# samuel-watson/glmmrMCML

Measured on AMD Instinct MI355X. Metric: MCML iters/sec x m chains (simlik evals/sec), higher is better.
Workload: dtype f64

## Files before the change

glmmrmcml_amd/csrc/dgemm_band.h:

```cpp
#pragma once
#include "dgemm_dlds.h"
#include "band_plan.h"

namespace mcml {

struct BandP {
    GemmP g;
    const BandItem* items;
    const int* wg_ptr;
    int nwg;
    double* part;
    int mode;
    unsigned long long* clocks;
};

static __global__ __launch_bounds__(256) void k_band_ranges(const double* A, int lda, int M, int K, int* krange)
{
    __shared__ int smin[256], smax[256];
    const int band = blockIdx.x, r0 = band * BD_BM;
    const int rows = (M - r0 < BD_BM) ? (M - r0) : BD_BM;
    int kmin = 1 << 30, kmax = -1;
    for (int k = threadIdx.x; k < K; k += 256) {
        const double* col = A + r0 + (size_t)k * lda;
        bool nz = false;
        for (int r = 0; r < rows; ++r) nz |= (col[r] != 0.0);
        if (nz) { kmin = min(kmin, k); kmax = max(kmax, k); }
    }
    smin[threadIdx.x] = kmin; smax[threadIdx.x] = kmax;
    __syncthreads();
    for (int o = 128; o > 0; o >>= 1) {
        if ((int)threadIdx.x < o) {
            smin[threadIdx.x] = min(smin[threadIdx.x], smin[threadIdx.x + o]);
            smax[threadIdx.x] = max(smax[threadIdx.x], smax[threadIdx.x + o]);
        }
        __syncthreads();
    }
    if (threadIdx.x == 0) {
        if (smax[0] < 0) { krange[2 * band] = 0; krange[2 * band + 1] = 0; }
        else { krange[2 * band] = smin[0] / BD_BK; krange[2 * band + 1] = smax[0] / BD_BK + 1; }
    }
}

#if defined(__HIP_DEVICE_COMPILE__)
#define BD_RD(dst, addr, off) asm volatile("ds_read_b64 %0, %1 offset:%2" : "=v"(dst) : "v"(addr), "i"(off))
#else
#define BD_RD(dst, addr, off) (dst = 0.0)
#endif
template <int KS, int NS>
__device__ __forceinline__ void bd_read(double (&a)[5], double (&b)[NS], unsigned aaddr, unsigned baddr)
{
    static_assert(NS == 1 || NS == 2, "one or two strips per wave");
    BD_RD(a[0], aaddr, KS * 4 * BD_BM * 8);
    BD_RD(a[1], aaddr, KS * 4 * BD_BM * 8 + 128);
    BD_RD(a[2], aaddr, KS * 4 * BD_BM * 8 + 256);
    BD_RD(a[3], aaddr, KS * 4 * BD_BM * 8 + 384);
    BD_RD(a[4], aaddr, KS * 4 * BD_BM * 8 + 512);
    BD_RD(b[0], baddr, KS * 2 * BD_BN * 16);
    if constexpr (NS == 2) BD_RD(b[1], baddr, KS * 2 * BD_BN * 16 + 256);
}
template <int LEAVE, int NS>
__device__ __forceinline__ void bd_wait(double (&a)[5], double (&b)[NS])
{
    static_assert(LEAVE == 0 || LEAVE == 5 + NS, "one substep's reads");
#if defined(__HIP_DEVICE_COMPILE__)
    if constexpr (NS == 1)
        asm volatile("s_waitcnt lgkmcnt(%[n])" : "+v"(a[0]), "+v"(a[1]), "+v"(a[2]), "+v"(a[3]), "+v"(a[4]), "+v"(b[0]) : [n] "n"(LEAVE));
    else
        asm volatile("s_waitcnt lgkmcnt(%[n])" : "+v"(a[0]), "+v"(a[1]), "+v"(a[2]), "+v"(a[3]), "+v"(a[4]), "+v"(b[0]), "+v"(b[1]) : [n] "n"(LEAVE));
#endif
}
template <int NS>
__device__ __forceinline__ void bd_mfma(d4 (&acc)[NS][5][1], const double (&a)[5], const double (&b)[NS])
{
#pragma unroll
    for (int j = 0; j < NS; ++j)
#pragma unroll
        for (int i = 0; i < 5; ++i) acc[j][i][0] = __builtin_amdgcn_mfma_f64_16x16x4f64(b[j], a[i], acc[j][i][0], 0, 0, 0);
}

__device__ __forceinline__ BandItem band_item(const BandItem* ip)
{
    BandItem item{0, 0, 0, -1};
#if defined(__HIP_DEVICE_COMPILE__)
    typedef int i4s __attribute__((ext_vector_type(4)));
    i4s raw;
    asm volatile("s_load_dwordx4 %0, %1, 0x0\n\ts_waitcnt lgkmcnt(0)" : "=&s"(raw) : "s"(ip) : "memory");
    item.band = raw.x; item.kt0 = raw.y; item.kt1 = raw.z; item.slot = raw.w;
#else
    item = *ip;
#endif
    return item;
}

template <int STRIDE, int NA, int NB>
struct BandFill {
    static constexpr int PER_TILE = NA + NB, A_CHUNKS = BD_A_BYTES / 1024;
    static_assert(STRIDE * NA >= A_CHUNKS && STRIDE * NB * 1024 == BD_B_BYTES, "the role's waves cover a stage");
    const GemmP& p;
    const BandItem* items;
    const int f, lane;
    const unsigned lds0;
    const size_t stepA;
    unsigned voa[NA], vob[NB];
    const char* sA = nullptr; const char* sB = nullptr;
    BandItem item{0, 0, 0, -1};

    __device__ __forceinline__ int a_rel(int s) const
    {
        return (STRIDE * NA > A_CHUNKS && f + STRIDE * s >= A_CHUNKS) ? STRIDE : STRIDE * s;
    }
    __device__ __forceinline__ BandFill(const BandP& bp, int f_, int lane_, int n0, unsigned lds0_)
        : p(bp.g), items(bp.items), f(f_), lane(lane_), lds0(lds0_), stepA((size_t)BD_BK * bp.g.lda * 8)
    {
#pragma unroll
        for (int s = 0; s < NB; ++s) {
            const int c = f + STRIDE * s;
            const int kp = c >> 1, n = ((c & 1) << 6) + lane;
            int gn = n0 + n;
            if (gn >= p.N) gn = 0;
            vob[s] = (unsigned)((2 * kp + (size_t)gn * p.ldb) * 8);
        }
    }
    __device__ __forceinline__ void load_item(int it)
    {
        item = band_item(items + it);
        const int m0 = item.band * BD_BM;
#pragma unroll
        for (int s = 0; s < NA; ++s) {
            const int o = (f + a_rel(s)) * 1024 + lane * 16;
            const int k = o / (BD_BM * 8), m = (o - k * BD_BM * 8) >> 3;
            int gm = m0 + m;
            if (gm >= p.M) gm = 0;
            voa[s] = (unsigned)((gm + (size_t)k * p.lda) * 8);
        }
        sA = reinterpret_cast<const char*>(p.A) + (size_t)item.kt0 * stepA;
        sB = reinterpret_cast<const char*>(p.B) + (size_t)item.kt0 * (BD_BK * 8);
    }
    __device__ __forceinline__ void issue(int stage)
    {
        const unsigned lbase = lds0 + stage * BD_STAGE_BYTES + f * 1024;
#pragma unroll
        for (int s = 0; s < NA; ++s) lds_dma16(lbase + a_rel(s) * 1024, voa[s], sA);
#pragma unroll
        for (int s = 0; s < NB; ++s) lds_dma16(lbase + BD_A_BYTES + STRIDE * s * 1024, vob[s], sB);
        sA += stepA;
        sB += BD_BK * 8;
    }
    __device__ __forceinline__ void wait_leave(int tiles) const
    {
        if (tiles >= 2) asm volatile("s_waitcnt vmcnt(%0)" :: "n"(2 * PER_TILE) : "memory");
        else if (tiles == 1) asm volatile("s_waitcnt vmcnt(%0)" :: "n"(PER_TILE) : "memory");
        else asm volatile("s_waitcnt vmcnt(0)" ::: "memory");
    }
};
struct BandNoFill {
    const BandItem* items;
    BandItem item{0, 0, 0, -1};
    __device__ __forceinline__ BandNoFill(const BandP& bp, int, int, int, unsigned) : items(bp.items) {}
    __device__ __forceinline__ void load_item(int it) { item = band_item(items + it); }
    __device__ __forceinline__ void issue(int) {}
    __device__ __forceinline__ void wait_leave(int) const {}
};
constexpr int BF_NA = 5, BF_NB = 8;

__device__ __forceinline__ void band_store_partial(double* tile, int strip, int lane, const d4 (&acc)[5][1])
{
    double* P = tile + (size_t)strip * (20 * 64) + lane;
#pragma unroll
    for (int i = 0; i < 5; ++i)
#pragma unroll
        for (int r = 0; r < 4; ++r) P[(i * 4 + r) * 64] = acc[i][0][r];
}

struct BandWg {
    int wave, lane, bj, it0, it1;
    __device__ __forceinline__ explicit BandWg(const BandP& bp)
    {
        const int tid = threadIdx.x;
        lane = tid & 63;
        wave = __builtin_amdgcn_readfirstlane(tid >> 6);
        const int nid = xcd_block_map(blockIdx.x, bp.nwg * bp.g.gn);
        const int pw = nid / bp.g.gn;
        bj = nid - pw * bp.g.gn;
        it0 = bp.wg_ptr[pw]; it1 = bp.wg_ptr[pw + 1];
    }
};

template <int NS, class Fill, bool DBG, class Epi>
__device__ __forceinline__ void band_walk(const BandP& bp, const Epi& epi, const BandWg& wg, int piece0, int strip0)
{
    constexpr int NJ = NS > 0 ? NS : 1;
    const GemmP& p = bp.g;
    extern __shared__ __attribute__((aligned(16))) double smem[];
    const unsigned lds0 = (unsigned)(size_t)(lds_ptr_t) reinterpret_cast<char*>(smem);
    const int lane = wg.lane, l15 = lane & 15, lk = lane >> 4;
    const int bj = wg.bj, n0 = bj * BD_BN, it0 = wg.it0, it1 = wg.it1;

    auto stamp = [&](int i) {
        if constexpr (DBG)
            if ((bp.mode & 16) && bp.clocks && threadIdx.x == 0)
                bp.clocks[8 + 8 * (size_t)blockIdx.x + i] = __builtin_amdgcn_s_memrealtime();
    };
    stamp(0);
    bool first_item = true;
    Fill fill(bp, piece0, lane, n0, lds0);
    bool pre = false;
    int issued = 0;
    if (it0 < it1) fill.load_item(it0);
    for (int it = it0; it < it1;) {
        const int band = fill.item.band, slot = fill.item.slot;
        const int nk = fill.item.kt1 - fill.item.kt0;

        d4 acc[NJ][5][1];
#pragma unroll
        for (int j = 0; j < NJ; ++j)
#pragma unroll
            for (int i = 0; i < 5; ++i) acc[j][i][0] = d4{0.0, 0.0, 0.0, 0.0};

        if (nk > 0) {
            const unsigned aoff = lds0 + lk * (BD_BM * 8) + l15 * 8;
            const unsigned boff = lds0 + BD_A_BYTES + (((lk >> 1) * BD_BN + strip0 * 16 + l15) << 4) + ((lk & 1) << 3);
            if (!pre) { issued = 0; for (; issued < BD_STAGES - 1 && issued < nk; ++issued) fill.issue(issued); }
            fill.wait_leave(issued - 1);
            __builtin_amdgcn_s_barrier();
            if (first_item) stamp(1);
            int st = 0;
            double ra[2][5], rb[2][NJ];
            if constexpr (NS > 0) bd_read<0>(ra[0], rb[0], aoff, boff);
            for (int kt = 0; kt < nk; ++kt) {
                if (issued < nk) {
                    int sn = st + BD_STAGES - 1; if (sn >= BD_STAGES) sn -= BD_STAGES;
                    fill.issue(sn);
                    ++issued;
                }
                const unsigned aaddr = aoff + st * BD_STAGE_BYTES, baddr = boff + st * BD_STAGE_BYTES;
                int stn = st + 1; if (stn >= BD_STAGES) stn = 0;
                if constexpr (NS > 0) {
#define BD_STEP(KS, CUR, NXT)                                   \
                    bd_read<KS + 1>(ra[NXT], rb[NXT], aaddr, baddr); \
                    bd_wait<5 + NS>(ra[CUR], rb[CUR]);               \
                    bd_mfma(acc, ra[CUR], rb[CUR]);                  \
                    __builtin_amdgcn_sched_barrier(0);
                    BD_STEP(0, 0, 1) BD_STEP(1, 1, 0) BD_STEP(2, 0, 1) BD_STEP(3, 1, 0)
                    BD_STEP(4, 0, 1) BD_STEP(5, 1, 0) BD_STEP(6, 0, 1)
#undef BD_STEP
                }
                fill.wait_leave(issued - kt - 2);
                if constexpr (NS > 0) bd_wait<0>(ra[1], rb[1]);
                __builtin_amdgcn_s_barrier();
                if constexpr (NS > 0) {
                    if (kt + 1 < nk) bd_read<0>(ra[0], rb[0], aoff + stn * BD_STAGE_BYTES, boff + stn * BD_STAGE_BYTES);
                    bd_mfma(acc, ra[1], rb[1]);
                    __builtin_amdgcn_sched_barrier(0);
                }
                st = stn;
            }
        }
        if (first_item) stamp(2);
        ++it;
        pre = false;
        if (it < it1) {
            fill.load_item(it);
            const int nkn = fill.item.kt1 - fill.item.kt0;
            if (nk > 0 && nkn > 0) {
                issued = 0;
                for (; issued < BD_STAGES - 1 && issued < nkn; ++issued) fill.issue(issued);
                pre = true;
            }
        }
        if constexpr (NS > 0) {
            if (slot < 0) {
                int elane = lane;
                if constexpr (NS > 1) asm volatile("" : "+v"(elane));
                epi(acc[0], band * BD_BM, n0 + strip0 * 16, elane, p.M, p.N, band);
                if constexpr (NS > 1) {
                    __builtin_amdgcn_sched_barrier(0);
                    epi(acc[1], band * BD_BM, n0 + strip0 * 16 + 16, elane, p.M, p.N, band);
                }
            } else {
                double* tile = bp.part + ((size_t)slot * p.gn + bj) * BD_TILE_ELEMS;
#pragma unroll
                for (int j = 0; j < NS; ++j) band_store_partial(tile, strip0 + j, lane, acc[j]);
            }
        }
        if (first_item) { stamp(3); first_item = false; }
        if (!pre) __builtin_amdgcn_s_barrier();
    }
    if constexpr (DBG)
        if ((bp.mode & 16) && bp.clocks) { asm volatile("s_waitcnt vmcnt(0)" ::: "memory"); stamp(4); }
}

template <class Epi, bool DBG>
__global__ __launch_bounds__(512) void dgemm_band_kernel(BandP bp, Epi epi)
{
    const BandWg wg(bp);
    unsigned long long t0c = 0, t0r = 0;
    if constexpr (DBG)
        if (bp.clocks && blockIdx.x == 0 && threadIdx.x == 0) { t0c = __builtin_amdgcn_s_memtime(); t0r = __builtin_amdgcn_s_memrealtime(); }
    band_walk<1, BandFill<8, BD_NA, BD_NB>, DBG>(bp, epi, wg, wg.wave, wg.wave);
    if constexpr (DBG)
        if (bp.clocks && blockIdx.x == 0 && threadIdx.x == 0) {
            atomicAdd(bp.clocks, __builtin_amdgcn_s_memtime() - t0c);
            atomicAdd(bp.clocks + 1, __builtin_amdgcn_s_memrealtime() - t0r);
        }
}

template <class Epi> struct BandFeed { static constexpr bool ok = false; };
template <> struct BandFeed<EpiAxpby> { static constexpr bool ok = true; };

static inline bool band_feed_enabled()
{
    const char* e = getenv("GLMMR_MCML_BAND_FEED");
    return !(e && !strcmp(e, "0"));
}

template <class Epi>
__global__ __launch_bounds__(512) void dgemm_band_feed_kernel(BandP bp, Epi epi)
{
    const BandWg wg(bp);
    if (wg.wave >= 4) band_walk<0, BandFill<4, BF_NA, BF_NB>, false>(bp, epi, wg, wg.wave - 4, 0);
    else band_walk<2, BandNoFill, false>(bp, epi, wg, 0, 2 * wg.wave);
}

template <class Epi>
__global__ __launch_bounds__(128) void k_band_reduce(const BandRed* red, const double* part, int gn, int M, int N, Epi epi)
{
    const BandRed rd = red[blockIdx.x];
    const int bj = blockIdx.y;
    const int lane = threadIdx.x & 63, wave = blockIdx.z * 2 + (threadIdx.x >> 6);
    d4 acc[5][1];
#pragma unroll
    for (int i = 0; i < 5; ++i) acc[i][0] = d4{0.0, 0.0, 0.0, 0.0};
    const size_t pstride = (size_t)gn * BD_TILE_ELEMS;
    const double* P0 = part + ((size_t)rd.s0 * gn + bj) * BD_TILE_ELEMS + (size_t)wave * (20 * 64) + lane;
    for (int s = rd.s0; s < rd.s1; s += 4) {
        double v[4][20];
#pragma unroll
        for (int u = 0; u < 4; ++u) {
            const double* P = P0 + (size_t)(s - rd.s0 + (s + u < rd.s1 ? u : 0)) * pstride;
#pragma unroll
            for (int t = 0; t < 20; ++t) v[u][t] = P[t * 64];
        }
#pragma unroll
        for (int u = 0; u < 4; ++u)
            if (s + u < rd.s1) {
#pragma unroll
                for (int i = 0; i < 5; ++i)
#pragma unroll
                    for (int r = 0; r < 4; ++r) acc[i][0][r] += v[u][i * 4 + r];
            }
    }
    epi(acc, rd.band * BD_BM, bj * BD_BN + wave * 16, lane, M, N, rd.band);
}

enum { BAND_FORM_AUTO = -1, BAND_FORM_8WAVE = 0, BAND_FORM_FEED = 1 };
template <class Epi, bool DBG = false>
static inline int launch_gemm_band(hipStream_t s, BandPlan& plan, int N, const double* A, int lda,
                                   const double* B, int ldb, const Epi& epi,
                                   unsigned long long* clocks = nullptr, int mode = 0, int form = BAND_FORM_AUTO,
                                   int* whole_band = nullptr)
{
    const int gn = (N + BD_BN - 1) / BD_BN;
    BandPlanDev* d = nullptr;
    MCML_TRY(plan.device_plan(gn, s, &d));
    BandP bp;
    bp.clocks = clocks;
    bp.mode = mode;
    bp.g = GemmP{plan.M, N, plan.K, A, lda, B, ldb, 0, gn, 0};
    bp.items = d->items.as<BandItem>();
    bp.wg_ptr = d->wg_ptr.as<int>();
    bp.nwg = d->nwg;
    bp.part = d->part.d();
    if (whole_band) *whole_band = d->paired;
    bool feed = false;
    if constexpr (BandFeed<Epi>::ok && !DBG) {
        feed = form == BAND_FORM_AUTO ? band_feed_enabled() : form == BAND_FORM_FEED;
        if (feed) {
            MCML_TRY(ensure_dynamic_lds(reinterpret_cast<const void*>(&dgemm_band_feed_kernel<Epi>), (int)BD_LDS_BYTES));
            hipLaunchKernelGGL((dgemm_band_feed_kernel<Epi>), dim3(d->nwg * gn), dim3(512), BD_LDS_BYTES, s, bp, epi);
        }
    }
    MCML_REQUIRE(feed || form != BAND_FORM_FEED, "launch_gemm_band: no feeder form of this instantiation");
    if (!feed) {
        MCML_TRY(ensure_dynamic_lds(reinterpret_cast<const void*>(&dgemm_band_kernel<Epi, DBG>), (int)BD_LDS_BYTES));
        hipLaunchKernelGGL((dgemm_band_kernel<Epi, DBG>), dim3(d->nwg * gn), dim3(512), BD_LDS_BYTES, s, bp, epi);
    }
    if (d->nred > 0)
        hipLaunchKernelGGL((k_band_reduce<Epi>), dim3(d->nred, gn, 4), dim3(128), 0, s, d->red.as<BandRed>(),
                           d->part.d(), gn, plan.M, N, epi);
    MCML_HIP(hipGetLastError());
    return MCML_OK;
}


}
```

glmmrmcml_amd/csrc/hmc.hip:

```cpp
#include <algorithm>
#include <atomic>
#include <chrono>
#include "entry.h"
#include "dgemm_mfma.h"
#include "dgemm_dlds.h"
#include "dgemm_band.h"
#include "dgemm_skinny.h"
#include "glm.h"
#include "reduce.h"
#include "rng.h"
#include "hmc_chain.h"
#include "hmc_cm.h"
#include "hmc_traj.h"

namespace mcml {

template <int FL>
struct EpiForwardT {
    double* MU; double* S; int ld; const double* xb; const double* y; int flink; int store_mu; double var_par;
    __device__ __forceinline__ double score(double yv, double mu) const {
        if constexpr (FL == 12) return glm_score_beta(yv, mu, var_par);
        else return glm_score(yv, mu, FL ? FL : flink);
    }
    __device__ __forceinline__ void elem(int m, int n, double accv) const {
        const double mu = xb[m] + accv;
        if (store_mu) MU[m + (size_t)n * ld] = mu;
        S[m + (size_t)n * ld] = score(y[m], mu);
    }
    template <int TM, int TN>
    __device__ __forceinline__ void operator()(d4 (&acc)[TM][TN], int mB, int nB, int lane, int M, int N,
                                               int) const {
        double xbv[TM], yv[TM];
#pragma unroll
        for (int i = 0; i < TM; ++i) {
            const int m = mB + 16 * i + (lane & 15);
            const int mm = m < M ? m : 0;
            xbv[i] = xb[mm]; yv[i] = y[mm];
        }
        double sc[TM][TN][4];
#pragma unroll
        for (int i = 0; i < TM; ++i)
#pragma unroll
            for (int j = 0; j < TN; ++j)
#pragma unroll
                for (int r = 0; r < 4; ++r) {
                    const double mu = xbv[i] + acc[i][j][r];
                    acc[i][j][r] = mu;
                    sc[i][j][r] = score(yv[i], mu);
                }
#pragma unroll
        for (int j = 0; j < TN; ++j)
#pragma unroll
            for (int r = 0; r < 4; ++r) {
                const int n = nB + 16 * j + (lane >> 4) + 4 * r;
                if (n >= N) continue;
#pragma unroll
                for (int i = 0; i < TM; ++i) {
                    const int m = mB + 16 * i + (lane & 15);
                    if (m < M) {
                        if (store_mu) MU[m + (size_t)n * ld] = acc[i][j][r];
                        S[m + (size_t)n * ld] = sc[i][j][r];
                    }
                }
            }
    }
};

struct EpiBackward {
    const double* Xs; double* G; double* R; double* UP; int ld;
    const double* e; const int* steps; int s; double post; int mode;
    __device__ __forceinline__ void elem(int m, int n, double accv) const {
        int st = 0; double en = 0.0;
        if (mode == 1) { st = steps[n]; en = e[n]; if (s >= st) return; }
        const size_t off = m + (size_t)n * ld;
        const double x = Xs[off];
        double g = -1.0 * x;
        g = g + post * accv;
        if (mode != 1 || s + 1 >= st) G[off] = g;
        if (mode == 1) {
            double rr = R[off];
            rr = rr + (en / 2) * g;
            if (s + 1 < st) {
                rr = rr + (en / 2) * g;
                UP[off] = x + en * rr;
            }
            R[off] = rr;
        }
    }
    template <int TM, int TN>
    __device__ __forceinline__ void operator()(d4 (&acc)[TM][TN], int mB, int nB, int lane, int M, int N,
                                               int) const {
#pragma unroll
        for (int j = 0; j < TN; ++j) {
            int stv[4]; double env[4]; bool inN[4]; size_t cb[4];
#pragma unroll
            for (int r = 0; r < 4; ++r) {
                const int n = nB + 16 * j + (lane >> 4) + 4 * r;
                inN[r] = n < N;
                const int nn = inN[r] ? n : 0;
                stv[r] = mode == 1 ? steps[nn] : 0;
                env[r] = mode == 1 ? e[nn] : 0.0;
                cb[r] = (size_t)nn * ld;
            }
            double xv[TM][4], rv[TM][4];
#pragma unroll
            for (int i = 0; i < TM; ++i) {
                const int m = mB + 16 * i + (lane & 15);
                const int mm = m < M ? m : 0;
#pragma unroll
                for (int r = 0; r < 4; ++r) {
                    xv[i][r] = Xs[mm + cb[r]];
                    rv[i][r] = mode == 1 ? R[mm + cb[r]] : 0.0;
                }
            }
#pragma unroll
            for (int r = 0; r < 4; ++r) {
                const double en = env[r];
                const bool more = s + 1 < stv[r];
#pragma unroll
                for (int i = 0; i < TM; ++i) {
                    const double x = xv[i][r];
                    double g = -1.0 * x;
                    g = g + post * acc[i][j][r];
                    acc[i][j][r] = g;
                    double rr = rv[i][r];
                    rr = rr + (en / 2) * g;
                    const double rr2 = rr + (en / 2) * g;
                    rr = more ? rr2 : rr;
                    rv[i][r] = rr;
                    xv[i][r] = x + en * rr;
                }
            }
#pragma unroll
            for (int r = 0; r < 4; ++r) {
                const bool act = inN[r] && (mode != 1 || s < stv[r]);
                if (!act) continue;
                const bool more = s + 1 < stv[r];
#pragma unroll
                for (int i = 0; i < TM; ++i) {
                    const int m = mB + 16 * i + (lane & 15);
                    if (m >= M) continue;
                    const size_t off = m + cb[r];
                    if (mode != 1 || !more) G[off] = acc[i][j][r];
                    if (mode == 1) {
                        if (more) UP[off] = xv[i][r];
                        R[off] = rv[i][r];
                    }
                }
            }
        }
    }
};

template <> struct BandFeed<EpiBackward> { static constexpr bool ok = true; };
template <> struct BandFeed<EpiForwardT<1>> { static constexpr bool ok = true; };
template <> struct BandFeed<EpiForwardT<3>> { static constexpr bool ok = true; };
template <> struct BandFeed<EpiForwardT<7>> { static constexpr bool ok = true; };


__global__ __launch_bounds__(256) void k_blockdiag_LV(int Q, int ncols, const int* start, const double* L, int ldl,
                                                      const double* V, int ldv, double* U, int ldu)
{
    const int q = blockIdx.x * 256 + threadIdx.x;
    if (q >= Q) return;
    const int s0 = start[q];
    for (int c = blockIdx.y; c < ncols; c += gridDim.y) {
        const double* v = V + (size_t)c * ldv;
        double acc = 0.0;
        for (int t = s0; t <= q; ++t) acc += L[q + (size_t)t * ldl] * v[t];
        U[q + (size_t)c * ldu] = acc;
    }
}

__global__ __launch_bounds__(256) void k_hmc_init(double* V, int ld, int Q, ChainArrays ca, uint64_t seed,
                                                  uint32_t chain_offset, uint32_t iter_idx, const double* inj_init)
{
    const int c = blockIdx.x;
    const uint32_t gid = chain_offset + (uint32_t)c;
    for (int q = threadIdx.x; q < Q; q += 256)
        V[q + (size_t)c * ld] = inj_init ? inj_init[q + (size_t)c * Q]
                                         : rng_normal(seed, (uint32_t)q, gid, 0u, 16u * iter_idx + 0u);
    if (threadIdx.x == 0) chain_reset(ca, c, seed, gid, iter_idx);
}

template <int FL>
__device__ __forceinline__ double chain_log_prob(const double* MU, int ldm, int n, const double* X, int ldx,
                                                 int Q, const double* y, double var_par, int flink_rt, int c,
                                                 double* sh)
{
    const int flink = FL ? FL : flink_rt;
    double ll = 0, lp = 0;
    for (int i0 = threadIdx.x; i0 < n; i0 += 1024) {
        double m4[4], y4[4];
#pragma unroll
        for (int u = 0; u < 4; ++u) {
            const int i = i0 + 256 * u;
            m4[u] = i < n ? MU[i + (size_t)c * ldm] : 0.0;
            y4[u] = i < n ? y[i] : 0.0;
        }
#pragma unroll
        for (int u = 0; u < 4; ++u)
            if (i0 + 256 * u < n) ll += glm_logpdf(y4[u], m4[u], var_par, flink);
    }
    for (int k0 = threadIdx.x; k0 < Q; k0 += 1024) {
        double x4[4];
#pragma unroll
        for (int u = 0; u < 4; ++u) { const int k = k0 + 256 * u; x4[u] = k < Q ? X[k + (size_t)c * ldx] : 0.0; }
#pragma unroll
        for (int u = 0; u < 4; ++u)
            if (k0 + 256 * u < Q) lp += glm_logpdf(x4[u], 0, 1, 7);
    }
    double a = block_sum(ll, sh);
    double b = block_sum(lp, sh);
    return a + b;
}

template <int FL>
__global__ __launch_bounds__(256) void k_hmc_lp0(const double* MU, int ldm, int n, const double* V, int ld, int Q,
                                                 const double* y, double var_par, int flink, double* lpcur)
{
    __shared__ double sh[4];
    double v = chain_log_prob<FL>(MU, ldm, n, V, ld, Q, y, var_par, flink, blockIdx.x, sh);
    if (threadIdx.x == 0) lpcur[blockIdx.x] = v;
}

__global__ __launch_bounds__(256) void k_hmc_propose(const double* V, const double* GRAD, double* R, double* UP,
                                                     int ld, int Q, ChainArrays ca, double lambda, int max_steps,
                                                     uint64_t seed, uint32_t chain_offset, uint32_t iter_idx,
                                                     int it, const double* inj_mom, int C)
{
    __shared__ double sh[4];
    const int c = blockIdx.x;
    const uint32_t gid = chain_offset + (uint32_t)c;
    const double e = ca.e[c];
    double ss = 0;
    for (int q = threadIdx.x; q < Q; q += 256) {
        const size_t off = q + (size_t)c * ld;
        double r = inj_mom ? inj_mom[q + ((size_t)it * C + c) * Q]
                           : rng_normal(seed, (uint32_t)q, gid, (uint32_t)it, 16u * iter_idx + 2u);
        ss += r * r;
        const double g = GRAD[off], v = V[off];
        r = r + (e / 2) * g;
        R[off] = r;
        UP[off] = v + e * r;
    }
    double tot = block_sum(ss, sh);
    if (threadIdx.x == 0) chain_begin_proposal(ca, c, tot, lambda, max_steps);
}

__global__ void k_max_steps(const int* steps, int C, int* out, unsigned long long* slot = nullptr, unsigned seq = 0)
{
    __shared__ int sh[256];
    int v = 0;
    for (int i = threadIdx.x; i < C; i += 256) v = max(v, steps[i]);
    sh[threadIdx.x] = v;
    __syncthreads();
    for (int o = 128; o > 0; o >>= 1) { if ((int)threadIdx.x < o) sh[threadIdx.x] = max(sh[threadIdx.x], sh[threadIdx.x + o]); __syncthreads(); }
    if (threadIdx.x == 0) {
        out[0] = sh[0];
        if (slot) __hip_atomic_store(slot, ((unsigned long long)seq << 32) | (unsigned)sh[0], __ATOMIC_RELEASE, __HIP_MEMORY_SCOPE_SYSTEM);
    }
}

template <int FL>
__global__ __launch_bounds__(256) void k_hmc_accept(double* V, double* GRAD, const double* R, const double* UP,
                                                    const double* GRADP, int ld, int Q, const double* MU, int ldm,
                                                    int n, const double* y, double var_par, int flink,
                                                    ChainArrays ca, double target_accept, int adapt, int it,
                                                    int C, uint8_t* flags, double* probs)
{
    __shared__ double sh[4];
    __shared__ int acc_s;
    const int c = blockIdx.x;
    double l2 = chain_log_prob<FL>(MU, ldm, n, UP, ld, Q, y, var_par, flink, c, sh);
    double kin = 0;
    for (int k0 = threadIdx.x; k0 < Q; k0 += 1024) {
        double r4[4];
#pragma unroll
        for (int u = 0; u < 4; ++u) { const int k = k0 + 256 * u; r4[u] = k < Q ? R[k + (size_t)c * ld] : 0.0; }
#pragma unroll
        for (int u = 0; u < 4; ++u)
            if (k0 + 256 * u < Q) kin += r4[u] * r4[u];
    }
    kin = block_sum(kin, sh);
    if (threadIdx.x == 0) acc_s = chain_decide(ca, c, l2, kin, target_accept, adapt, it, C, flags, probs);
    __syncthreads();
    const int acc = acc_s;
    if (acc)
        for (int k0 = threadIdx.x; k0 < Q; k0 += 1024) {
            double u4[4], g4[4];
#pragma unroll
            for (int u = 0; u < 4; ++u) {
                const int k = k0 + 256 * u;
                const size_t off = (k < Q ? k : 0) + (size_t)c * ld;
                u4[u] = UP[off]; g4[u] = GRADP[off];
            }
#pragma unroll
            for (int u = 0; u < 4; ++u) {
                const int k = k0 + 256 * u;
                if (k < Q) { const size_t off = k + (size_t)c * ld; V[off] = u4[u]; GRAD[off] = g4[u]; }
            }
        }
}

__global__ __launch_bounds__(256) void k_hmc_store(const double* V, int ld, int Q, double* SAMP, int lds,
                                                   int stride, int col)
{
    const int c = blockIdx.x;
    for (int k = threadIdx.x; k < Q; k += 256) SAMP[k + (size_t)(c * stride + col) * lds] = V[k + (size_t)c * ld];
}

__global__ void k_hmc_diag(ChainArrays ca, int C, double* out)
{
    if (threadIdx.x != 0 || blockIdx.x != 0) return;
    double sa = 0, se = 0, mn = 1e300, mx = 0, ms = 0, sl = 0;
    for (int c = 0; c < C; ++c) {
        sa += ca.acc[c]; se += ca.e[c];
        mn = fmin(mn, ca.e[c]); mx = fmax(mx, ca.e[c]);
        ms = fmax(ms, (double)ca.steps[c]); sl += (double)ca.leap[c];
    }
    out[0] = sa; out[1] = se; out[2] = mn; out[3] = mx; out[4] = ms; out[5] = sl;
}

static bool cm_traj_used(const Ctx& c) { return c.traj_mode == 1 && c.sp.active && c.cp.ready && c.cp.plan.feasible; }

static std::atomic<long long> g_traj_launches{0};
long long cm_traj_launch_count() { return g_traj_launches.load(); }

static int cm_traj_launch(Ctx& c, const TrajArgs& a)
{
    const CompView m = comp_view(c);
    const int waves = cp_waves(c.cp.plan, cp_forced_waves(CP_TRAJ_WAVES_ENV));
    const int lds = cp_lds_bytes(m.max_vars, waves);
    const dim3 grid(m.nitems, cm_chain_blocks(a.C));
    MCML_TRY((dispatch_flink<1, 3, 7, 12>(c.flink, [&](auto FL) {
        if (waves == 4) {
            MCML_TRY(ensure_dynamic_lds((const void*)k_cm_traj<FL(), 4>, cp_lds_bytes(CP_MAX_VARS, 4)));
            hipLaunchKernelGGL((k_cm_traj<FL(), 4>), grid, dim3(256), lds, c.stream, m, a);
        } else {
            MCML_TRY(ensure_dynamic_lds((const void*)k_cm_traj<FL(), 1>, cp_lds_bytes(CP_MAX_VARS, 1)));
            hipLaunchKernelGGL((k_cm_traj<FL(), 1>), grid, dim3(64), lds, c.stream, m, a);
        }
        return (int)MCML_OK;
    })));
    MCML_HIP(hipGetLastError());
    ++g_traj_launches;
    return MCML_OK;
}

static int hmc_alloc(Ctx& c, int C)
{
    HmcState& h = c.hmc;
    h.C = C; h.Cw = C;
    h.cm = c.sp.active;
    auto mat = [&](DevMat& m, int len) { return h.cm ? m.alloc(C, len) : m.alloc(len, C); };
    for (DevMat* m : {&h.V, &h.R, &h.UP, &h.GRAD, &h.GRADP}) MCML_TRY(mat(*m, c.Q));
    MCML_TRY(mat(h.MU, c.n)); MCML_TRY(mat(h.S, c.n));
    MCML_TRY(h.chain.ensure(sizeof(double) * (size_t)round_up(C, 16) * 8));
    if (h.cm) {
        const size_t nchn = (size_t)(c.n + CM_ROWS - 1) / CM_ROWS, nchq = (size_t)(c.Q + cm_qrows(c.Q) - 1) / cm_qrows(c.Q);
        MCML_TRY(h.cm_part.ensure(sizeof(double) * (nchn + 3 * nchq + 4) * (size_t)h.V.ld));
        MCML_TRY(h.cm_acc.ensure(sizeof(int) * (size_t)round_up(C, 64)));
        if (c.sp.factored) { MCML_TRY(h.LX.alloc(C, c.Q)); MCML_TRY(h.ZS.alloc(C, c.Q)); }
        if (cm_traj_used(c)) MCML_TRY(h.cp_part.ensure(sizeof(double) * 4 * (size_t)c.cp.plan.nitems() * h.V.ld));
        return MCML_OK;
    }
    MCML_HIP(hipMemsetAsync(h.V.d(), 0, sizeof(double) * (size_t)h.V.ld * C, c.stream));
    MCML_HIP(hipMemsetAsync(h.UP.d(), 0, sizeof(double) * (size_t)h.UP.ld * C, c.stream));
    MCML_HIP(hipMemsetAsync(h.S.d(), 0, sizeof(double) * (size_t)h.S.ld * C, c.stream));
    return MCML_OK;
}

static bool use_dlds()
{
    static int v = -1;
    if (v < 0) { const char* e = getenv("GLMMR_MCML_GEMM"); v = (e && !strcmp(e, "reg")) ? 0 : 1; }
    return v == 1;
}

static bool use_skinny()
{
    const char* e = getenv("GLMMR_MCML_SKINNY");
    return !(e && !strcmp(e, "0"));
}

struct DenseOp { BandPlan& plan; bool band; int M, K; const DevMat& A; };
template <class Epi>
static int dense_product(Ctx& c, int dir, const DenseOp& a, const double* B, int ldb, const Epi& epi)
{
    const int N = c.hmc.Cw, lda = a.A.ld;
    const double* A = a.A.d();
    if (use_skinny() && skinny_applicable(a.plan, a.M, a.K, N, lda)) {
        c.last_kernel[dir] = KERNEL_SKINNY;
        return launch_skinny(c.stream, a.plan, N, A, lda, B, ldb, epi);
    }
    if (a.band && dlds_applicable(a.M, N, a.K, A, lda, a.A.cols_alloc, B, ldb)) {
        c.last_kernel[dir] = KERNEL_BAND;
        return launch_gemm_band(c.stream, a.plan, N, A, lda, B, ldb, epi);
    }
    if (use_dlds() && dlds_applicable(a.M, N, a.K, A, lda, a.A.cols_alloc, B, ldb)) {
        c.last_kernel[dir] = KERNEL_DLDS;
        return launch_gemm_dlds(c.stream, a.M, N, a.K, A, lda, B, ldb, epi);
    }
    c.last_kernel[dir] = KERNEL_REG;
    return launch_gemm<false>(c.stream, a.M, N, a.K, A, lda, B, ldb, epi);
}

enum : unsigned {
    PROD_STORE_MU = 1,
    PROD_CHAIN = 2,
    PROD_WANT_LL = 4,
    PROD_LX_READY = 8,
};

static int hmc_forward(Ctx& c, const double* X, int ldx, double var_par, unsigned flags = PROD_STORE_MU)
{
    HmcState& h = c.hmc;
    const int store_mu = (flags & PROD_STORE_MU) ? 1 : 0;
    const int slot = c.prof.begin(c.stream, 0, (flags & PROD_CHAIN) != 0);
    int rc;
    if (h.cm) {
        c.last_kernel[0] = KERNEL_SPARSE;
        const int rpw = CM_FR;
        dim3 grid((c.n + 4 * rpw - 1) / (4 * rpw), (h.Cw + 63) / 64);
        int W = c.sp.W; const int* col = c.sp.ell_col.as<int>(); const double* val = c.sp.ell_val.d(); const double* Xin = X;
        if (c.sp.factored) {
            if (!(flags & PROD_LX_READY))
            hipLaunchKernelGGL(k_cm_Lrow, dim3((c.Q + 3) / 4, (h.Cw + 63) / 64), dim3(256), 0, c.stream, c.Q, h.Cw, h.V.ld,
                               c.sp.row_start.as<int>(), c.L.d(), c.L.ld, X, h.LX.d());
            W = c.z_width; col = c.z_idx.as<int>(); val = c.z_val.d(); Xin = h.LX.d();
        }
        double* pll = nullptr;
        if (flags & PROD_WANT_LL) {
            MCML_TRY(h.cm_part_fwd.ensure(sizeof(double) * (size_t)grid.x * h.V.ld));
            pll = h.cm_part_fwd.d();
        }
        dispatch_flink<1, 3, 7, 12>(c.flink, [&](auto FL) {
            hipLaunchKernelGGL((k_cm_forward<FL()>), grid, dim3(256), 0, c.stream, c.n, h.Cw, h.V.ld, W, col, val, Xin, c.xb.d(),
                               c.y.d(), c.flink, var_par, store_mu, h.MU.d(), h.S.d(), rpw, pll, h.V.ld);
        });
        rc = (hipGetLastError() == hipSuccess) ? MCML_OK : MCML_EHIP;
    } else
        rc = dispatch_flink<1, 3, 7, 12>(c.flink, [&](auto FL) {
            return dense_product(c, 0, DenseOp{c.plan_fwd, c.band_fwd, c.n, c.Q, c.ZL}, X, ldx,
                                 EpiForwardT<FL()>{h.MU.d(), h.S.d(), h.MU.ld, c.xb.d(), c.y.d(), c.flink, store_mu, var_par});
        });
    c.prof.end(c.stream, slot);
    return rc;
}

static int hmc_backward(Ctx& c, const double* Xs, double* G, int s, double var_par, int mode, unsigned flags = 0,
                        int next_lx = 0)
{
    HmcState& h = c.hmc;
    ChainArrays ca = chain_arrays(h);
    EpiBackward epi{Xs, G, h.R.d(), h.UP.d(), h.V.ld, ca.e, ca.steps, s, glm_score_post(var_par, c.flink), mode};
    const int slot = c.prof.begin(c.stream, 1, (flags & PROD_CHAIN) != 0);
    int rc;
    if (h.cm) {
        const bool f = c.sp.factored;
// ... 431 lines not shown
```

Baseline: 1230.

## Prefetch band GEMM epilogue operands during the final K tile

Splits the forward and backward epilogues into a load phase and a finish phase. The load parts (xb/y, or Xs/R/steps/e) are interleaved with the MFMA substeps of the last K tile, so their global-memory latency is hidden behind compute instead of sitting after the loop. It adds register pressure and code complexity. Falls back to the old path when prefetch is disabled, for example the backward epilogue outside mode 1. The 32-bit offset path is used only when the address range fits.

```diff
diff --git a/glmmrmcml_amd/csrc/dgemm_band.h b/glmmrmcml_amd/csrc/dgemm_band.h
--- a/glmmrmcml_amd/csrc/dgemm_band.h
+++ b/glmmrmcml_amd/csrc/dgemm_band.h
@@ -1,4 +1,5 @@
 #pragma once
+#include <type_traits>
 #include "dgemm_dlds.h"
 #include "band_plan.h"
 
@@ -172,6 +173,27 @@
         for (int r = 0; r < 4; ++r) P[(i * 4 + r) * 64] = acc[i][0][r];
 }
 
+template <class Epi> struct EpiSplit { static constexpr bool ok = false; };
+template <class Epi, bool OK = EpiSplit<Epi>::ok> struct BandEpiIn {
+    struct type {};
+    static constexpr int parts = 0;
+    static constexpr bool per_item = false;
+};
+template <class Epi> struct BandEpiIn<Epi, true> {
+    using type = typename Epi::template In<5>;
+    static constexpr int parts = Epi::template LOAD_PARTS<5>;
+    static constexpr bool per_item = Epi::IN_PER_ITEM;
+    static_assert(parts >= 1 && parts <= 7, "one part per substep in front of a K tile's barrier");
+};
+
+template <int P, class Epi>
+__device__ __forceinline__ void band_epi_load(const Epi& epi, typename BandEpiIn<Epi>::type& in, int mB, int nB, int lane,
+                                              int M, int N)
+{
+    epi.template load_part<P, false>(in, mB, nB, lane, M, N);
+    if constexpr (P + 1 < BandEpiIn<Epi>::parts) band_epi_load<P + 1>(epi, in, mB, nB, lane, M, N);
+}
+
 struct BandWg {
     int wave, lane, bj, it0, it1;
     __device__ __forceinline__ explicit BandWg(const BandP& bp)
@@ -190,6 +212,8 @@
 __device__ __forceinline__ void band_walk(const BandP& bp, const Epi& epi, const BandWg& wg, int piece0, int strip0)
 {
     constexpr int NJ = NS > 0 ? NS : 1;
+    constexpr bool PF = NS == 2 && std::is_same<Fill, BandNoFill>::value && EpiSplit<Epi>::ok;
+    constexpr int EPI_PARTS = BandEpiIn<Epi>::parts;
     const GemmP& p = bp.g;
     extern __shared__ __attribute__((aligned(16))) double smem[];
     const unsigned lds0 = (unsigned)(size_t)(lds_ptr_t) reinterpret_cast<char*>(smem);
@@ -216,6 +240,9 @@
         for (int j = 0; j < NJ; ++j)
 #pragma unroll
             for (int i = 0; i < 5; ++i) acc[j][i][0] = d4{0.0, 0.0, 0.0, 0.0};
+        int elane = lane;
+        [[maybe_unused]] typename BandEpiIn<Epi>::type ein;
+        bool pf = false;
 
         if (nk > 0) {
             const unsigned aoff = lds0 + lk * (BD_BM * 8) + l15 * 8;
@@ -227,23 +254,24 @@
             int st = 0;
             double ra[2][5], rb[2][NJ];
             if constexpr (NS > 0) bd_read<0>(ra[0], rb[0], aoff, boff);
-            for (int kt = 0; kt < nk; ++kt) {
-                if (issued < nk) {
-                    int sn = st + BD_STAGES - 1; if (sn >= BD_STAGES) sn -= BD_STAGES;
-                    fill.issue(sn);
-                    ++issued;
-                }
-                const unsigned aaddr = aoff + st * BD_STAGE_BYTES, baddr = boff + st * BD_STAGE_BYTES;
-                int stn = st + 1; if (stn >= BD_STAGES) stn = 0;
-                if constexpr (NS > 0) {
 #define BD_STEP(KS, CUR, NXT)                                   \
                     bd_read<KS + 1>(ra[NXT], rb[NXT], aaddr, baddr); \
                     bd_wait<5 + NS>(ra[CUR], rb[CUR]);               \
                     bd_mfma(acc, ra[CUR], rb[CUR]);                  \
                     __builtin_amdgcn_sched_barrier(0);
+            if constexpr (PF) pf = slot < 0 && epi.prefetch(p.M, p.N);
+            const int nloop = pf ? nk - 1 : nk;
+            for (int kt = 0; kt < nloop; ++kt) {
+                if (issued < nk) {
+                    int sn = st + BD_STAGES - 1; if (sn >= BD_STAGES) sn -= BD_STAGES;
+                    fill.issue(sn);
+                    ++issued;
+                }
+                const unsigned aaddr = aoff + st * BD_STAGE_BYTES, baddr = boff + st * BD_STAGE_BYTES;
+                int stn = st + 1; if (stn >= BD_STAGES) stn = 0;
+                if constexpr (NS > 0) {
                     BD_STEP(0, 0, 1) BD_STEP(1, 1, 0) BD_STEP(2, 0, 1) BD_STEP(3, 1, 0)
                     BD_STEP(4, 0, 1) BD_STEP(5, 1, 0) BD_STEP(6, 0, 1)
-#undef BD_STEP
                 }
                 fill.wait_leave(issued - kt - 2);
                 if constexpr (NS > 0) bd_wait<0>(ra[1], rb[1]);
@@ -255,6 +283,30 @@
                 }
                 st = stn;
             }
+            if constexpr (PF) {
+                if (__builtin_expect(pf, 1)) {
+                    asm volatile("" : "+v"(elane));
+                    const int mB = band * BD_BM, nB = n0 + strip0 * 16;
+                    const unsigned aaddr = aoff + st * BD_STAGE_BYTES, baddr = boff + st * BD_STAGE_BYTES;
+#define BD_LD(KS) if constexpr (KS < EPI_PARTS) \
+                        epi.template load_part<(KS < EPI_PARTS ? KS : 0), true>(ein, mB, nB, elane, p.M, p.N);
+#define BD_STEP_LD(KS, CUR, NXT)                                \
+                    bd_read<KS + 1>(ra[NXT], rb[NXT], aaddr, baddr); \
+                    bd_wait<5 + NS>(ra[CUR], rb[CUR]);               \
+                    bd_mfma(acc, ra[CUR], rb[CUR]);                  \
+                    BD_LD(KS) \
+                    __builtin_amdgcn_sched_barrier(0);
+                    BD_STEP_LD(0, 0, 1) BD_STEP_LD(1, 1, 0) BD_STEP_LD(2, 0, 1) BD_STEP_LD(3, 1, 0)
+                    BD_STEP_LD(4, 0, 1) BD_STEP_LD(5, 1, 0) BD_STEP_LD(6, 0, 1)
+#undef BD_STEP_LD
+                    bd_wait<0>(ra[1], rb[1]);
+                    __builtin_amdgcn_s_barrier();
+                    bd_mfma(acc, ra[1], rb[1]);
+                    __builtin_amdgcn_sched_barrier(0);
+                }
+            }
+#undef BD_LD
+#undef BD_STEP
         }
         if (first_item) stamp(2);
         ++it;
@@ -270,12 +322,20 @@
         }
         if constexpr (NS > 0) {
             if (slot < 0) {
-                int elane = lane;
                 if constexpr (NS > 1) asm volatile("" : "+v"(elane));
-                epi(acc[0], band * BD_BM, n0 + strip0 * 16, elane, p.M, p.N, band);
+                if constexpr (PF) {
+                    if (__builtin_expect(!pf, 0)) band_epi_load<0>(epi, ein, band * BD_BM, n0 + strip0 * 16, elane, p.M, p.N);
+                    epi.finish(acc[0], ein, band * BD_BM, n0 + strip0 * 16, elane, p.M, p.N);
+                } else {
+                    epi(acc[0], band * BD_BM, n0 + strip0 * 16, elane, p.M, p.N, band);
+                }
                 if constexpr (NS > 1) {
                     __builtin_amdgcn_sched_barrier(0);
-                    epi(acc[1], band * BD_BM, n0 + strip0 * 16 + 16, elane, p.M, p.N, band);
+                    if (pf && BandEpiIn<Epi>::per_item) {
+                        if constexpr (PF) epi.finish(acc[1], ein, band * BD_BM, n0 + strip0 * 16 + 16, elane, p.M, p.N);
+                    } else {
+                        epi(acc[1], band * BD_BM, n0 + strip0 * 16 + 16, elane, p.M, p.N, band);
+                    }
                 }
             } else {
                 double* tile = bp.part + ((size_t)slot * p.gn + bj) * BD_TILE_ELEMS;
diff --git a/glmmrmcml_amd/csrc/hmc.hip b/glmmrmcml_amd/csrc/hmc.hip
--- a/glmmrmcml_amd/csrc/hmc.hip
+++ b/glmmrmcml_amd/csrc/hmc.hip
@@ -63,6 +63,46 @@
                     }
                 }
             }
+    }
+    template <int TM> struct In { double xbv[TM], yv[TM]; };
+    template <int TM> static constexpr int LOAD_PARTS = 1;
+    static constexpr bool IN_PER_ITEM = true;
+    __device__ __forceinline__ bool prefetch(int, int) const { return true; }
+    template <int P, bool NARROW, int TM>
+    __device__ __forceinline__ void load_part(In<TM>& in, int mB, int, int lane, int M, int) const {
+        static_assert(P == 0, "one part");
+#pragma unroll
+        for (int i = 0; i < TM; ++i) {
+            const int m = mB + 16 * i + (lane & 15);
+            const int mm = m < M ? m : 0;
+            in.xbv[i] = xb[mm]; in.yv[i] = y[mm];
+        }
+    }
+    template <int TM>
+    __device__ __forceinline__ void finish(d4 (&acc)[TM][1], const In<TM>& in, int mB, int nB, int lane, int M,
+                                           int N) const {
+        double sc[TM][4];
+#pragma unroll
+        for (int i = 0; i < TM; ++i)
+#pragma unroll
+            for (int r = 0; r < 4; ++r) {
+                const double mu = in.xbv[i] + acc[i][0][r];
+                acc[i][0][r] = mu;
+                sc[i][r] = score(in.yv[i], mu);
+            }
+#pragma unroll
+        for (int r = 0; r < 4; ++r) {
+            const int n = nB + (lane >> 4) + 4 * r;
+            if (n >= N) continue;
+#pragma unroll
+            for (int i = 0; i < TM; ++i) {
+                const int m = mB + 16 * i + (lane & 15);
+                if (m < M) {
+                    if (store_mu) MU[m + (size_t)n * ld] = acc[i][0][r];
+                    S[m + (size_t)n * ld] = sc[i][r];
+                }
+            }
+        }
     }
 };
 
@@ -150,12 +190,94 @@
             }
         }
     }
+    template <int TM> struct In { double xv[TM][4], rv[TM][4]; int stv[4]; double env[4]; };
+    template <int TM> static constexpr int LOAD_PARTS = TM + 1;
+    static constexpr bool IN_PER_ITEM = false;
+    __device__ __forceinline__ bool prefetch(int M, int N) const {
+        return mode == 1 && ((size_t)ld * N + M) * 8 < 0xffffffffull;
+    }
+    template <int P, bool NARROW, int TM>
+    __device__ __forceinline__ void load_part(In<TM>& in, int mB, int nB, int lane, int M, int N) const {
+        static_assert(P >= 0 && P <= TM, "the columns, then TM row groups");
+        int nn[4];
+#pragma unroll
+        for (int r = 0; r < 4; ++r) {
+            const int n = nB + (lane >> 4) + 4 * r;
+            nn[r] = n < N ? n : 0;
+        }
+        if constexpr (P == 0) {
+#pragma unroll
+            for (int r = 0; r < 4; ++r) {
+                in.stv[r] = mode == 1 ? steps[nn[r]] : 0;
+                in.env[r] = mode == 1 ? e[nn[r]] : 0.0;
+            }
+        } else {
+            constexpr int i = P - 1;
+            const int m = mB + 16 * i + (lane & 15);
+            const int mm = m < M ? m : 0;
+#pragma unroll
+            for (int r = 0; r < 4; ++r) {
+                const size_t off64 = (mm + (size_t)nn[r] * ld) * 8;
+                const std::conditional_t<NARROW, unsigned, size_t> off = off64;
+                in.xv[i][r] = *reinterpret_cast<const double*>(reinterpret_cast<const char*>(Xs) + off);
+                in.rv[i][r] = mode == 1 ? *reinterpret_cast<const double*>(reinterpret_cast<const char*>(R) + off) : 0.0;
+            }
+        }
+    }
+    template <int TM>
+    __device__ __forceinline__ void finish(d4 (&acc)[TM][1], In<TM>& in, int mB, int nB, int lane, int M,
+                                           int N) const {
+        bool inN[4]; size_t cb[4];
+#pragma unroll
+        for (int r = 0; r < 4; ++r) {
+            const int n = nB + (lane >> 4) + 4 * r;
+            inN[r] = n < N;
+            cb[r] = (size_t)(inN[r] ? n : 0) * ld;
+        }
+#pragma unroll
+        for (int r = 0; r < 4; ++r) {
+            const double en = in.env[r];
+            const bool more = s + 1 < in.stv[r];
+#pragma unroll
+            for (int i = 0; i < TM; ++i) {
+                const double x = in.xv[i][r];
+                double g = -1.0 * x;
+                g = g + post * acc[i][0][r];
+                acc[i][0][r] = g;
+                double rr = in.rv[i][r];
+                rr = rr + (en / 2) * g;
+                const double rr2 = rr + (en / 2) * g;
+                rr = more ? rr2 : rr;
+                in.rv[i][r] = rr;
+                in.xv[i][r] = x + en * rr;
+            }
+        }
+#pragma unroll
+        for (int r = 0; r < 4; ++r) {
+            const bool act = inN[r] && (mode != 1 || s < in.stv[r]);
+            if (!act) continue;
+            const bool more = s + 1 < in.stv[r];
+#pragma unroll
+            for (int i = 0; i < TM; ++i) {
+                const int m = mB + 16 * i + (lane & 15);
+                if (m >= M) continue;
+                const size_t off = m + cb[r];
+                if (mode != 1 || !more) G[off] = acc[i][0][r];
+                if (mode == 1) {
+                    if (more) UP[off] = in.xv[i][r];
+                    R[off] = in.rv[i][r];
+                }
+            }
+        }
+    }
 };
 
 template <> struct BandFeed<EpiBackward> { static constexpr bool ok = true; };
 template <> struct BandFeed<EpiForwardT<1>> { static constexpr bool ok = true; };
 template <> struct BandFeed<EpiForwardT<3>> { static constexpr bool ok = true; };
 template <> struct BandFeed<EpiForwardT<7>> { static constexpr bool ok = true; };
+template <> struct EpiSplit<EpiBackward> { static constexpr bool ok = true; };
+template <int FL> struct EpiSplit<EpiForwardT<FL>> { static constexpr bool ok = true; };
 
 
 __global__ __launch_bounds__(256) void k_blockdiag_LV(int Q, int ncols, const int* start, const double* L, int ldl,
```

After: 1238, median of 6. Within noise of the previous version (+0.6%).

## Hand off second epilogue strip from MFMA waves to feeder waves via LDS

Applied to the files above, without the earlier changes.

In the feeder-form band GEMM kernel, each MFMA wave now writes its second 16-column accumulator strip into a spare LDS stage, and the paired feeder wave reads it back and runs that strip's epilogue or partial store. The aim is to split epilogue work between the compute and loader waves instead of leaving it all on the MFMA waves. To keep the hand-off stage free, the feeder defers its prefetch issue until after the epilogue. The cost is an extra barrier, an LDS round trip per item, and a later prefetch start for the next item.

```diff
diff --git a/glmmrmcml_amd/csrc/dgemm_band.h b/glmmrmcml_amd/csrc/dgemm_band.h
--- a/glmmrmcml_amd/csrc/dgemm_band.h
+++ b/glmmrmcml_amd/csrc/dgemm_band.h
@@ -186,10 +186,18 @@
     }
 };
 
-template <int NS, class Fill, bool DBG, class Epi>
+enum { BD_HAND_NONE = 0, BD_HAND_GIVE = 1, BD_HAND_TAKE = 2 };
+constexpr int BD_HAND_STAGE = 2;
+static_assert(4 * 64 * 20 * 8 <= BD_STAGE_BYTES, "four strips of 20 doubles per lane fit the hand-off stage");
+static_assert(BD_HAND_STAGE == BD_STAGES - 1, "`pre` fills the stages below the hand-off stage only");
+
+template <int NS, class Fill, bool DBG, int HAND = BD_HAND_NONE, class Epi>
 __device__ __forceinline__ void band_walk(const BandP& bp, const Epi& epi, const BandWg& wg, int piece0, int strip0)
 {
+    static_assert(HAND == BD_HAND_NONE || (HAND == BD_HAND_GIVE && NS == 2) || (HAND == BD_HAND_TAKE && NS == 0),
+                  "the MFMA wave of a pair gives its second strip, the feeder takes it");
     constexpr int NJ = NS > 0 ? NS : 1;
+    constexpr int NE = HAND != BD_HAND_NONE ? 1 : NS;
     const GemmP& p = bp.g;
     extern __shared__ __attribute__((aligned(16))) double smem[];
     const unsigned lds0 = (unsigned)(size_t)(lds_ptr_t) reinterpret_cast<char*>(smem);
@@ -264,25 +272,50 @@
             const int nkn = fill.item.kt1 - fill.item.kt0;
             if (nk > 0 && nkn > 0) {
                 issued = 0;
-                for (; issued < BD_STAGES - 1 && issued < nkn; ++issued) fill.issue(issued);
+                if constexpr (HAND != BD_HAND_TAKE)
+                    for (; issued < BD_STAGES - 1 && issued < nkn; ++issued) fill.issue(issued);
                 pre = true;
             }
         }
-        if constexpr (NS > 0) {
+        if constexpr (HAND != BD_HAND_NONE) {
+            double* hand = smem + (BD_HAND_STAGE * BD_STAGE_BYTES) / 8 + (strip0 >> 1) * (20 * 64) + lane;
+            if constexpr (HAND == BD_HAND_GIVE) {
+#pragma unroll
+                for (int i = 0; i < 5; ++i)
+#pragma unroll
+                    for (int r = 0; r < 4; ++r) hand[(i * 4 + r) * 64] = acc[1][i][0][r];
+                asm volatile("s_waitcnt lgkmcnt(0)" ::: "memory");
+                __builtin_amdgcn_s_barrier();
+            } else {
+                __builtin_amdgcn_s_barrier();
+                asm volatile("" ::: "memory");
+#pragma unroll
+                for (int i = 0; i < 5; ++i)
+#pragma unroll
+                    for (int r = 0; r < 4; ++r) acc[0][i][0][r] = hand[(i * 4 + r) * 64];
+                asm volatile("s_waitcnt lgkmcnt(0)" ::: "memory");
+            }
+        }
+        if constexpr (NE > 0) {
             if (slot < 0) {
                 int elane = lane;
-                if constexpr (NS > 1) asm volatile("" : "+v"(elane));
+                if constexpr (NS > 1 || HAND != BD_HAND_NONE) asm volatile("" : "+v"(elane));
                 epi(acc[0], band * BD_BM, n0 + strip0 * 16, elane, p.M, p.N, band);
-                if constexpr (NS > 1) {
+                if constexpr (NE > 1) {
                     __builtin_amdgcn_sched_barrier(0);
                     epi(acc[1], band * BD_BM, n0 + strip0 * 16 + 16, elane, p.M, p.N, band);
                 }
             } else {
                 double* tile = bp.part + ((size_t)slot * p.gn + bj) * BD_TILE_ELEMS;
 #pragma unroll
-                for (int j = 0; j < NS; ++j) band_store_partial(tile, strip0 + j, lane, acc[j]);
-            }
-        }
+                for (int j = 0; j < NE; ++j) band_store_partial(tile, strip0 + j, lane, acc[j]);
+            }
+        }
+        if constexpr (HAND == BD_HAND_TAKE)
+            if (pre) {
+                const int nkn = fill.item.kt1 - fill.item.kt0;
+                for (; issued < BD_STAGES - 1 && issued < nkn; ++issued) fill.issue(issued);
+            }
         if (first_item) { stamp(3); first_item = false; }
         if (!pre) __builtin_amdgcn_s_barrier();
     }
@@ -307,6 +340,8 @@
 
 template <class Epi> struct BandFeed { static constexpr bool ok = false; };
 template <> struct BandFeed<EpiAxpby> { static constexpr bool ok = true; };
+template <class Epi> struct BandHandoff { static constexpr bool ok = false; };
+template <> struct BandHandoff<EpiAxpby> { static constexpr bool ok = true; };
 
 static inline bool band_feed_enabled()
 {
@@ -318,8 +353,12 @@
 __global__ __launch_bounds__(512) void dgemm_band_feed_kernel(BandP bp, Epi epi)
 {
     const BandWg wg(bp);
-    if (wg.wave >= 4) band_walk<0, BandFill<4, BF_NA, BF_NB>, false>(bp, epi, wg, wg.wave - 4, 0);
-    else band_walk<2, BandNoFill, false>(bp, epi, wg, 0, 2 * wg.wave);
+    static_assert(BandFeed<Epi>::ok || !BandHandoff<Epi>::ok, "the hand-off is a property of a feeder-form instantiation");
+    constexpr bool H = BandHandoff<Epi>::ok;
+    if (wg.wave >= 4)
+        band_walk<0, BandFill<4, BF_NA, BF_NB>, false, H ? BD_HAND_TAKE : BD_HAND_NONE>(bp, epi, wg, wg.wave - 4,
+                                                                                         H ? 2 * wg.wave - 7 : 0);
+    else band_walk<2, BandNoFill, false, H ? BD_HAND_GIVE : BD_HAND_NONE>(bp, epi, wg, 0, 2 * wg.wave);
 }
 
 template <class Epi>
diff --git a/glmmrmcml_amd/csrc/hmc.hip b/glmmrmcml_amd/csrc/hmc.hip
--- a/glmmrmcml_amd/csrc/hmc.hip
+++ b/glmmrmcml_amd/csrc/hmc.hip
@@ -156,6 +156,10 @@
 template <> struct BandFeed<EpiForwardT<1>> { static constexpr bool ok = true; };
 template <> struct BandFeed<EpiForwardT<3>> { static constexpr bool ok = true; };
 template <> struct BandFeed<EpiForwardT<7>> { static constexpr bool ok = true; };
+template <> struct BandHandoff<EpiBackward> { static constexpr bool ok = true; };
+template <> struct BandHandoff<EpiForwardT<1>> { static constexpr bool ok = true; };
+template <> struct BandHandoff<EpiForwardT<3>> { static constexpr bool ok = true; };
+template <> struct BandHandoff<EpiForwardT<7>> { static constexpr bool ok = true; };
 
 
 __global__ __launch_bounds__(256) void k_blockdiag_LV(int Q, int ncols, const int* start, const double* L, int ldl,
```

Result: no change. 1218 before, 1223 after (median of 3 runs) (+0.4%).
